# ErickRosete/tacorl

Measured on AMD Instinct MI355X. Metric: offline grad-steps/sec (batch=256, 84x84 RGB), higher is better.
Workload: dtype bf16; 1 GPU; tacorl actor-critic training_step, frozen LMP (BASELINE configs[1]); per_gpu_batch=256, global_batch=256, window=16, image=84x84x3, frames=fp32 CHW (reference batch schema), latent_plan=16, n_action_samples=4, phase=Q (epoch>=bc_epochs), action_decoder_loss=every step (reference behaviour), parallelism=dp1, hip_graph=True, losses_finite=True

## Files before the change

tacorl_amd/csrc/mlp_fused.hip:

```cpp
#include "mlp_fused.h"

#include <stdlib.h>

#include "common.h"

namespace {

constexpr int BMF = 32;
constexpr int MTF = BMF / 16;
constexpr int XP = 272;
constexpr int MAXD = 256;
constexpr int MF_NT = 1024, MF_CW = MAXD / (MF_NT / 64), MF_NTW = MF_CW / 16;

struct MlpXSeg { const float* p; int ld, c0, mod, pad; };
struct MlpFwdArgs {
  MlpXSeg seg[MF_MAXP][MF_MAXSEG];
  int nseg[MF_MAXP];
  float* xw[MF_MAXP];
  const float* x[MF_MAXP];
  const float* params[MF_MAXP];
  const __bf16* pbf[MF_MAXP];
  float* act[MF_MAXP];
  int M[MF_MAXP];
  long zoff[MF_MAXP][MF_MAXL], yoff[MF_MAXP][MF_MAXL];
// ... 375 lines not shown
                if (col + r < KO) o[r] = v[r];
            }
          }
          *reinterpret_cast<bf16x4*>(xout + row * XP + col) = bf16x4{(__bf16)v[0], (__bf16)v[1], (__bf16)v[2], (__bf16)v[3]};
        }
      }
    }
    lds_barrier();
    cur ^= 1;
  }
}
__global__ __launch_bounds__(MF_NT) void mlp_fused_bwd_kernel(MlpBwdArgs a) { mlp_fused_bwd_body<32>(a); }
__global__ __launch_bounds__(MF_NT) void mlp_fused_bwd_big_kernel(MlpBwdArgs a) { mlp_fused_bwd_body<64>(a); }

constexpr int WG_MS = 2048;
constexpr int WG_MT = 32;
constexpr int WG_TP = 40;
constexpr int WG_OPB = 256 * WG_TP * 2;

struct MlpWgArgs {
  const float* x[MF_MAXP];
  const float* act[MF_MAXP];
  const float* dlast[MF_MAXP];
  const float* dz[MF_MAXP];
  float* slab[MF_MAXP];
  int M[MF_MAXP];
  long yoff[MF_MAXP][MF_MAXL], dzoff[MF_MAXP][MF_MAXL];
  int acts[MF_MAXL];
  long sloff[MF_MAXL];
  long rec;
  int dims[MF_MAXL + 1];
  int L, ldx, ldo, ms;
};

__device__ __forceinline__ float wg_dpp1(float x) {
  return __builtin_bit_cast(float, __builtin_amdgcn_mov_dpp(__builtin_bit_cast(int, x), 0xB1, 0xF, 0xF, true));
}
__device__ __forceinline__ float wg_dpp2(float x) {
  return __builtin_bit_cast(float, __builtin_amdgcn_mov_dpp(__builtin_bit_cast(int, x), 0x4E, 0xF, 0xF, true));
}
__device__ __forceinline__ void wg_quad_transpose(f32x4& v, int q) {
  const bool o1 = q & 1, o2 = q & 2;
  const float x0 = wg_dpp1(o1 ? v[0] : v[1]), x1 = wg_dpp1(o1 ? v[2] : v[3]);
  if (o1) { v[0] = x0; v[2] = x1; } else { v[1] = x0; v[3] = x1; }
  const float y0 = wg_dpp2(o2 ? v[0] : v[2]), y1 = wg_dpp2(o2 ? v[1] : v[3]);
  if (o2) { v[0] = y0; v[1] = y1; } else { v[2] = y0; v[3] = y1; }
}

__global__ __launch_bounds__(512) void mlp_wgrad_fused_kernel(MlpWgArgs a) {
  extern __shared__ __attribute__((aligned(16))) unsigned char smem[];
  const int p = blockIdx.z, l = blockIdx.y, m0 = blockIdx.x * a.ms, M = a.M[p];
  if (m0 >= M) return;
  const int tid = threadIdx.x, lane = tid & 63, w = tid >> 6, i = lane & 15, g = lane >> 4, q = tid & 3;
  const int qd = (tid >> 2) & 63, jh = tid >> 8;
  const int K = a.dims[l], N = a.dims[l + 1];
  const long yo = l == 0 ? 0 : a.yoff[p][l - 1];
  const float* X = l == 0 ? a.x[p] : a.act[p] + (yo < 0 ? -(yo + 1) : yo);
  const int actX = l > 0 && yo < 0 ? a.acts[l - 1] : ACT_NONE;
  const int ldX = l == 0 ? a.ldx : K;
  const float* Z = l == a.L - 1 ? a.dlast[p] : a.dz[p] + a.dzoff[p][l];
  const int ldZ = l == a.L - 1 ? a.ldo : N;
  const bool vecX = (ldX & 3) == 0 && (K & 3) == 0 && ((uintptr_t)X & 15) == 0;
  const bool vecZ = (ldZ & 3) == 0 && (N & 3) == 0 && ((uintptr_t)Z & 15) == 0;
  const int KT = (K + 15) >> 4, NT = (N + 15) >> 4;
  const int mend = min(M, m0 + a.ms), nsteps = (mend - m0 + WG_MT - 1) / WG_MT;

  f32x4 rx[4], rz[4];
  auto fetch = [&](const float* S, int ld, int C, bool vec, int mt, f32x4 (&r)[4]) {
    const int c = 4 * qd;
#pragma unroll
    for (int j = 0; j < 4; j++) {
      const int m = m0 + mt * WG_MT + 4 * (2 * j + jh) + q;
      const bool rok = m < mend;
      const float* src = S + (long)(rok ? m : m0) * ld;
      if (vec) {
        const f32x4 v = *reinterpret_cast<const f32x4*>(src + (c < C ? c : 0));
        const bool ok = rok && c < C;
        r[j] = f32x4{ok ? v[0] : 0.f, ok ? v[1] : 0.f, ok ? v[2] : 0.f, ok ? v[3] : 0.f};
      } else {
#pragma unroll
        for (int e = 0; e < 4; e++) {
          const float v = src[c + e < C ? c + e : 0];
          r[j][e] = rok && c + e < C ? v : 0.f;
        }
      }
    }
  };
  auto stash = [&](f32x4 (&r)[4], unsigned char* T, int act) {
#pragma unroll
    for (int j = 0; j < 4; j++) {
      f32x4 v = r[j];
      if (act != ACT_NONE) v = f32x4{act_fast(act, v[0]), act_fast(act, v[1]), act_fast(act, v[2]), act_fast(act, v[3])};
      wg_quad_transpose(v, q);
      *reinterpret_cast<bf16x4*>(T + ((4 * qd + q) * WG_TP + 4 * (2 * j + jh)) * 2) = bf16x4{(__bf16)v[0], (__bf16)v[1], (__bf16)v[2], (__bf16)v[3]};
    }
  };
  f32x4 acc[2][17];
#pragma unroll
  for (int nt = 0; nt < 2; nt++)
#pragma unroll
    for (int kt = 0; kt < 17; kt++) acc[nt][kt] = f32x4{0.f, 0.f, 0.f, 0.f};
  const __bf16 one = (__bf16)1.0f;
  const bf16x8 ones = {one, one, one, one, one, one, one, one};

  fetch(X, ldX, K, vecX, 0, rx);
  fetch(Z, ldZ, N, vecZ, 0, rz);
  for (int s = 0; s < nsteps; s++) {
    unsigned char* TX = smem + (s & 1) * 2 * WG_OPB;
    unsigned char* TZ = TX + WG_OPB;
    stash(rx, TX, actX);
    stash(rz, TZ, ACT_NONE);
    __syncthreads();
    if (s + 1 < nsteps) { fetch(X, ldX, K, vecX, s + 1, rx); fetch(Z, ldZ, N, vecZ, s + 1, rz); }
    bf16x8 zf[2];
#pragma unroll
    for (int nt = 0; nt < 2; nt++)
      zf[nt] = *reinterpret_cast<const bf16x8*>(TZ + ((16 * (w + 8 * nt) + i) * WG_TP + 8 * g) * 2);
#pragma unroll
    for (int kt = 0; kt < 16; kt++) {
      if (kt < KT) {
        const bf16x8 xf = *reinterpret_cast<const bf16x8*>(TX + ((16 * kt + i) * WG_TP + 8 * g) * 2);
#pragma unroll
        for (int nt = 0; nt < 2; nt++)
          if (w + 8 * nt < NT) acc[nt][kt] = __builtin_amdgcn_mfma_f32_16x16x32_bf16(xf, zf[nt], acc[nt][kt], 0, 0, 0);
      }
    }
#pragma unroll
    for (int nt = 0; nt < 2; nt++)
      if (w + 8 * nt < NT) acc[nt][16] = __builtin_amdgcn_mfma_f32_16x16x32_bf16(ones, zf[nt], acc[nt][16], 0, 0, 0);
  }
  float* rec = a.slab[p] + (long)blockIdx.x * a.rec + a.sloff[l];
  const bool vecK = (K & 3) == 0;
#pragma unroll
  for (int nt = 0; nt < 2; nt++) {
    const int n = 16 * (w + 8 * nt) + i;
    if (w + 8 * nt >= NT || n >= N) continue;
#pragma unroll
    for (int kt = 0; kt < 16; kt++) {
      const int k = 16 * kt + 4 * g;
      if (kt < KT) {
        if (vecK) {
          if (k < K) *reinterpret_cast<f32x4*>(rec + (long)n * K + k) = acc[nt][kt];
        } else {
#pragma unroll
          for (int r = 0; r < 4; r++)
            if (k + r < K) rec[(long)n * K + k + r] = acc[nt][kt][r];
        }
      }
    }
    if (g == 0) rec[(long)N * K + n] = acc[nt][16][0];
  }
}

struct MlpWgReduceArgs {
  const float* slab[MF_MAXP];
  float* grad[MF_MAXP];
  int nslice[MF_MAXP];
  long sloff[MF_MAXL], woff[MF_MAXL], boff[MF_MAXL];
  long rec;
  int dims[MF_MAXL + 1];
  int accumulate;
};
__global__ __launch_bounds__(256) void mlp_wgrad_reduce_kernel(MlpWgReduceArgs a) {
  const int l = blockIdx.y, p = blockIdx.z, K = a.dims[l], N = a.dims[l + 1], ns = a.nslice[p];
  const long nw = (long)N * K, tot = nw + N;
  const float* __restrict__ s0 = a.slab[p] + a.sloff[l];
  float* __restrict__ gr = a.grad[p];
  for (long e = (long)blockIdx.x * 256 + threadIdx.x; e < tot; e += (long)gridDim.x * 256) {
    float t = 0.f;
#pragma unroll 8
    for (int s = 0; s < ns; s++) t += s0[(long)s * a.rec + e];
    float* d = gr + (e < nw ? a.woff[l] + e : a.boff[l] + (e - nw));
    *d = a.accumulate ? *d + t : t;
  }
}

#define RED_MAXJ 8
struct MlpWgReduceMulti {
  MlpWgReduceArgs job[RED_MAXJ];
  int gx[RED_MAXJ], L[RED_MAXJ], first[RED_MAXJ + 1];
  int njob;
};
__global__ __launch_bounds__(256) void mlp_wgrad_reduce_multi_kernel(MlpWgReduceMulti m) {
  int j = 0;
#pragma unroll
  for (int t = 1; t < RED_MAXJ; t++) j = (t < m.njob && (int)blockIdx.z >= m.first[t]) ? t : j;
  const int gx = m.gx[j];
  if ((int)blockIdx.y >= m.L[j] || (int)blockIdx.x >= gx) return;
  const MlpWgReduceArgs& a = m.job[j];
  const int l = blockIdx.y, p = blockIdx.z - m.first[j], K = a.dims[l], N = a.dims[l + 1], ns = a.nslice[p];
  const long nw = (long)N * K, tot = nw + N;
  const float* __restrict__ s0 = a.slab[p] + a.sloff[l];
  float* __restrict__ gr = a.grad[p];
  for (long e = (long)blockIdx.x * 256 + threadIdx.x; e < tot; e += (long)gx * 256) {
    float t = 0.f;
#pragma unroll 8
    for (int s = 0; s < ns; s++) t += s0[(long)s * a.rec + e];
    float* d = gr + (e < nw ? a.woff[l] + e : a.boff[l] + (e - nw));
    *d = a.accumulate ? *d + t : t;
  }
}
struct RedState { bool on = false; MlpWgReduceMulti m{}; };
thread_local RedState g_red;
int red_flush(hipStream_t st) {
  MlpWgReduceMulti& m = g_red.m;
  if (m.njob == 0) return 0;
  int gx = 1, Ly = 1;
  for (int j = 0; j < m.njob; j++) { gx = m.gx[j] > gx ? m.gx[j] : gx; Ly = m.L[j] > Ly ? m.L[j] : Ly; }
  hipLaunchKernelGGL(mlp_wgrad_reduce_multi_kernel, dim3(gx, Ly, m.first[m.njob]), dim3(256), 0, st, m);
  m.njob = 0; m.first[0] = 0;
  return hipGetLastError() == hipSuccess ? 0 : -1;
}
int launch_reduce(const MlpWgReduceArgs& r, int gx, int Ly, int nprob, hipStream_t st) {
  if (!g_red.on) {
    hipLaunchKernelGGL(mlp_wgrad_reduce_kernel, dim3(gx, Ly, nprob), dim3(256), 0, st, r);
    return hipGetLastError() == hipSuccess ? 0 : -1;
  }
  MlpWgReduceMulti& m = g_red.m;
  if (m.njob == RED_MAXJ) {
    hipLaunchKernelGGL(mlp_wgrad_reduce_kernel, dim3(gx, Ly, nprob), dim3(256), 0, st, r);
    return hipGetLastError() == hipSuccess ? 0 : -1;
  }
  m.job[m.njob] = r; m.gx[m.njob] = gx; m.L[m.njob] = Ly; m.first[m.njob + 1] = m.first[m.njob] + nprob;
  m.njob++;
  return 0;
}

typedef _Float16 f16x4 __attribute__((ext_vector_type(4)));
#ifdef MLP_STAMPS
__device__ unsigned long long g_mlp_stamps[2][64];
#define MLP_STAMP(k, j) do { if (stamp_on) g_mlp_stamps[k][j] = clock64(); } while (0)
#else
#define MLP_STAMP(k, j) do { } while (0)
#endif

struct MlpBigFwdArgs {
  MlpXSeg seg[MF_MAXP][MF_MAXSEG];
  int nseg[MF_MAXP];
  float* xw[MF_MAXP];
  const float* x[MF_MAXP];
  const float* params[MF_MAXP];
  const __bf16* pbf[MF_MAXP];
  float* act[MF_MAXP];
  int M[MF_MAXP];
  long ybf[MF_MAXP][MF_MAXL], sbf[MF_MAXP][MF_MAXL];
  long yout[MF_MAXP];
  long woff[MF_MAXL], boff[MF_MAXL];
  int dims[MF_MAXL + 1], acts[MF_MAXL];
  int L, ldx;
  int dbg;
};

template <int BMF_>
__device__ __forceinline__ void mlp_big_fwd_body(const MlpBigFwdArgs& a) {
  constexpr int BMF = BMF_, MTF = BMF / 16;
  extern __shared__ __attribute__((aligned(16))) unsigned char smem[];
  __bf16* X = reinterpret_cast<__bf16*>(smem);
  const int p = blockIdx.y, m0 = blockIdx.x * BMF, M = a.M[p];
  const int Mp = (M + 63) & ~63;
  if (m0 >= Mp) return;
  const int tid = threadIdx.x, lane = tid & 63, w = tid >> 6, i = lane & 15, g = lane >> 4;
  const int n0 = MF_CW * w;
#ifdef MLP_STAMPS
  const bool stamp_on = blockIdx.x == 300 && p == 0 && tid == 0;
#endif
  MLP_STAMP(0, 0);
  const int K0 = a.dims[0], c8 = (K0 + 7) / 8;
  f32x4 xr[2][2];
  const float* x = a.x[p];
  const int ns = a.nseg[p];
#pragma unroll
  for (int u = 0; u < 2; u++) {
    const int c = tid + u * MF_NT, row = c / c8, k = (c - row * c8) * 8;
    const bool ok = c < BMF * c8 && m0 + row < M;
    if (ns > 0) {
      int sg = 0;
#pragma unroll
      for (int t = 1; t < MF_MAXSEG; t++) sg = (t < ns && k >= a.seg[p][t].c0) ? t : sg;
      const MlpXSeg s = a.seg[p][sg];
      const int cend = sg + 1 < ns ? a.seg[p][sg + 1].c0 : K0;
      const int r = s.mod ? (m0 + row) % s.mod : m0 + row;
      const float* q = s.p + (ok ? (long)r * s.ld + (k - s.c0) : 0);
      if (ok && k + 8 <= cend) { xr[u][0] = *reinterpret_cast<const f32x4*>(q); xr[u][1] = *reinterpret_cast<const f32x4*>(q + 4); }
      else {
#pragma unroll
        for (int j = 0; j < 4; j++) { xr[u][0][j] = ok && k + j < cend ? q[j] : 0.f; xr[u][1][j] = ok && k + 4 + j < cend ? q[4 + j] : 0.f; }
      }
      continue;
    }
    const float* q = x + (ok ? (long)(m0 + row) * a.ldx + k : 0);
    if (ok && k + 8 <= a.ldx) { xr[u][0] = *reinterpret_cast<const f32x4*>(q); xr[u][1] = *reinterpret_cast<const f32x4*>(q + 4); }
    else {
#pragma unroll
      for (int j = 0; j < 4; j++) { xr[u][0][j] = ok && k + j < K0 ? q[j] : 0.f; xr[u][1][j] = ok && k + 4 + j < K0 ? q[4 + j] : 0.f; }
    }
  }
  bf16x8 B[8][MF_NTW];
  auto load_layer = [&](int l) {
    const int K = a.dims[l], N = a.dims[l + 1];
    const __bf16* Wb = a.pbf[p] + a.woff[l];
#pragma unroll
    for (int ks = 0; ks < 8; ks++)
#pragma unroll
      for (int nt = 0; nt < MF_NTW; nt++) B[ks][nt] = load_w(Wb, K, N, n0 + 16 * nt + i, 32 * ks + 8 * g);
  };
  if (n0 < a.dims[1]) load_layer(0);
// ... 857 lines not shown
      if (k + 8 <= a.ldx && (a.ldx & 3) == 0) {
        const f32x4 lo = *reinterpret_cast<const f32x4*>(q), hi = *reinterpret_cast<const f32x4*>(q + 4);
#pragma unroll
        for (int j = 0; j < 4; j++) { v[j] = (__bf16)(k + j < K0 ? lo[j] : 0.f); v[4 + j] = (__bf16)(k + 4 + j < K0 ? hi[j] : 0.f); }
      } else {
#pragma unroll
        for (int j = 0; j < 8; j++)
          if (k + j < K0) v[j] = (__bf16)q[j];
      }
    }
    *reinterpret_cast<bf16x8*>(o + (long)row * 128 + k) = v;
  }
}

constexpr int OUT_RPW = 512;
struct MlpWgOutArgs {
  const __bf16* y[MF_MAXP]; const float* dlast[MF_MAXP]; float* slab[MF_MAXP];
  int M[MF_MAXP];
  long rec;
  int NL, ldo, rpw;
};
__global__ __launch_bounds__(256) void mlp_wgrad_out_kernel(MlpWgOutArgs a) {
  __shared__ float red[8][4][256 + 1];
  const int p = blockIdx.y, M = a.M[p], r0 = blockIdx.x * a.rpw;
  if (r0 >= M) return;
  const int r1 = min(M, r0 + a.rpw), tid = threadIdx.x, cg = tid & 31, rg = tid >> 5, NL = a.NL;
  float acc[4][8], bsum[4];
#pragma unroll
  for (int n = 0; n < 4; n++) {
    bsum[n] = 0.f;
#pragma unroll
    for (int j = 0; j < 8; j++) acc[n][j] = 0.f;
  }
  const __bf16* __restrict__ y = a.y[p];
  const float* __restrict__ d = a.dlast[p];
  for (int rb = r0 + rg; rb < r1; rb += 32) {
    bf16x8 v[4];
    float dv[4][4];
#pragma unroll
    for (int u = 0; u < 4; u++) {
      const int r = rb + 8 * u, rc = r < r1 ? r : r0;
      v[u] = *reinterpret_cast<const bf16x8*>(y + (long)rc * 256 + 8 * cg);
#pragma unroll
      for (int n = 0; n < 4; n++) dv[u][n] = (n < NL && r < r1) ? (float)(__bf16)d[(long)rc * a.ldo + n] : 0.f;
    }
#pragma unroll
    for (int u = 0; u < 4; u++)
#pragma unroll
      for (int n = 0; n < 4; n++)
        if (n < NL) {
          bsum[n] += dv[u][n];
#pragma unroll
          for (int j = 0; j < 8; j++) acc[n][j] += dv[u][n] * (float)v[u][j];
        }
  }
#pragma unroll
  for (int n = 0; n < 4; n++) {
#pragma unroll
    for (int j = 0; j < 8; j++) red[rg][n][8 * cg + j] = acc[n][j];
    if (cg == 0) red[rg][n][256] = bsum[n];
  }
  __syncthreads();
  float* rec = a.slab[p] + (long)blockIdx.x * a.rec;
  for (int e = tid; e < NL * 257; e += 256) {
    const int n = e / 257, k = e - n * 257;
    float t = 0.f;
#pragma unroll
    for (int g8 = 0; g8 < 8; g8++) t += red[g8][n][k];
    if (k < 256) rec[(long)n * 256 + k] = t; else rec[(long)NL * 256 + n] = t;
  }
}

}

namespace {
struct PrepState {
  bool on = false;
  PrepMultiArgs a{};
  int nprob[PREP_MAXS] = {};
};
thread_local PrepState g_prep;
int prep_flush(hipStream_t st) {
  PrepMultiArgs& a = g_prep.a;
  if (a.nsite == 0 && a.ncv == 0) return TACORL_OK;
  int maxL = 1;
  for (int s = 0; s < a.nsite; s++) maxL = a.site[s].L > maxL ? a.site[s].L : maxL;
  hipLaunchKernelGGL(prep_multi_kernel, dim3(64, maxL, a.first[a.nsite] + a.ncv), dim3(256), 0, st, a);
  a.nsite = 0; a.ncv = 0; a.first[0] = 0;
  return hipGetLastError() == hipSuccess ? TACORL_OK : TACORL_ELAUNCH;
}
}
bool prep_deferring() { return g_prep.on; }
int prep_defer_wtpack(const WtPackArgs& k, int nprob, hipStream_t st) {
  PrepMultiArgs& a = g_prep.a;
  if (a.nsite == PREP_MAXS) { const int rc = prep_flush(st); if (rc != TACORL_OK) return rc; }
  a.site[a.nsite] = k;
  a.first[a.nsite + 1] = a.first[a.nsite] + nprob;
  a.nsite++;
  return TACORL_OK;
}
int prep_defer_bf16(const float* src, void* dst, long count, hipStream_t st) {
  PrepMultiArgs& a = g_prep.a;
  if (a.ncv == PREP_MAXB) { const int rc = prep_flush(st); if (rc != TACORL_OK) return rc; }
  a.csrc[a.ncv] = src; a.cdst[a.ncv] = (__bf16*)dst; a.cn4[a.ncv] = count / 4;
  a.ncv++;
  return TACORL_OK;
}
extern "C" int tacorl_reduce_batch_begin(void) {
  if (g_red.on) return TACORL_EINVAL;
  g_red.on = true;
  g_red.m.njob = 0; g_red.m.first[0] = 0;
  return TACORL_OK;
}
extern "C" int tacorl_reduce_batch_end(void* stream) {
  if (!g_red.on) return TACORL_EINVAL;
  g_red.on = false;
  return red_flush((hipStream_t)stream) ? TACORL_ELAUNCH : TACORL_OK;
}
extern "C" int tacorl_prep_batch_begin(void) {
  if (g_prep.on) return TACORL_EINVAL;
  g_prep.on = true;
  g_prep.a.nsite = 0; g_prep.a.ncv = 0; g_prep.a.first[0] = 0;
  return TACORL_OK;
}
extern "C" int tacorl_prep_batch_end(void* stream) {
  if (!g_prep.on) return TACORL_EINVAL;
  g_prep.on = false;
  return prep_flush((hipStream_t)stream);
}


bool mlp_fused_wgrad_ok(int nprob, int L, const int* dims) {
  if (nprob < 1 || nprob > MF_MAXP || L < 1 || L > MF_MAXL) return false;
  for (int l = 0; l <= L; l++)
    if (dims[l] < 1 || dims[l] > MAXD) return false;
  return true;
}
static long mlp_wgrad_record(int L, const int* dims, long* sloff) {
  long off = 0;
  for (int l = 0; l < L; l++) {
    if (sloff) sloff[l] = off;
    off += (long)dims[l + 1] * dims[l] + dims[l + 1];
    off = (off + 3) & ~3L;
  }
  return off;
}
static int mlp_wgrad_rows(int nprob, const int* M, int L) {
  long rows = 0;
  for (int p = 0; p < nprob; p++) rows += M[p] > 0 ? M[p] : 0;
  long ms = rows * L / 128;
  ms = (ms + WG_MT - 1) / WG_MT * WG_MT;
  return (int)(ms < WG_MT ? WG_MT : ms > WG_MS ? WG_MS : ms);
}
size_t mlp_fused_wgrad_slab_floats(int nprob, const int* M, int L, const int* dims) {
  const long rec = mlp_wgrad_record(L, dims, nullptr);
  const int ms = mlp_wgrad_rows(nprob, M, L);
  size_t tot = 0;
  for (int p = 0; p < nprob; p++) tot += (size_t)((M[p] + ms - 1) / ms) * rec;
  return tot;
}
int mlp_fused_wgrad(int nprob, const float* const* x, int ldx, const float* const* act, const float* const* d_out, int ldo,
                    const float* const* dz, float* const* grads, float* slab, const int* M, int L, const int* dims,
                    const long* yoff, const long* dzoff, const long* woff, const long* boff, int accumulate, hipStream_t st,
                    const int* acts) {
  MlpWgArgs a{};
  MlpWgReduceArgs r{};
  a.rec = r.rec = mlp_wgrad_record(L, dims, a.sloff);
  a.L = L; a.ldx = ldx; a.ldo = ldo; r.accumulate = accumulate;
  {
    int Mg[MF_MAXP], n = 0;
    for (int p = 0; p < nprob; p++) Mg[n++] = M[p];
    a.ms = mlp_wgrad_rows(n, Mg, L);
  }
  for (int l = 0; l <= L; l++) a.dims[l] = r.dims[l] = dims[l];
  for (int l = 0; l < L; l++) { r.sloff[l] = a.sloff[l]; r.woff[l] = woff[l]; r.boff[l] = boff[l]; a.acts[l] = acts ? acts[l] : ACT_NONE; }
  int n2 = 0, maxs = 0;
  float* sp = slab;
  for (int p = 0; p < nprob; p++) {
    if (!grads[p] || M[p] <= 0) continue;
    const int ns = (M[p] + a.ms - 1) / a.ms;
    a.x[n2] = x[p]; a.act[n2] = act[p]; a.dlast[n2] = d_out[p]; a.dz[n2] = dz[p]; a.M[n2] = M[p]; a.slab[n2] = sp;
    r.slab[n2] = sp; r.grad[n2] = grads[p]; r.nslice[n2] = ns;
    for (int l = 0; l < L; l++) { a.yoff[n2][l] = yoff[p * MF_MAXL + l]; a.dzoff[n2][l] = dzoff[p * MF_MAXL + l]; }
    sp += (size_t)ns * a.rec;
    maxs = ns > maxs ? ns : maxs;
    n2++;
  }
  if (!n2) return 0;
  static int once = hipFuncSetAttribute(reinterpret_cast<const void*>(mlp_wgrad_fused_kernel),
                                        hipFuncAttributeMaxDynamicSharedMemorySize, 4 * WG_OPB) == hipSuccess ? 0 : -1;
  if (once) return -1;
  hipLaunchKernelGGL(mlp_wgrad_fused_kernel, dim3(maxs, L, n2), dim3(512), 4 * WG_OPB, st, a);
  if (launch_reduce(r, 256, L, n2, st)) return -1;
  return hipGetLastError() == hipSuccess ? 0 : -1;
}

static int mlp_big_rows() {
  static const int v = [] { const char* e = getenv("TACORL_MLP_BIG_ROWS"); return e ? atoi(e) : 2048; }();
  return v;
}
bool mlp_big_prob_ok(int M, int L, const int* dims, const int* acts) {
  static const int on = [] { const char* e = getenv("TACORL_MLP_BIG"); return e ? atoi(e) : 1; }();
  if (!on || L < 2 || L > MF_MAXL || M < mlp_big_rows()) return false;
  if (dims[0] < 8 || dims[0] > 128 || dims[L] < 1 || dims[L] > 4) return false;
  for (int l = 1; l < L; l++)
    if (dims[l] != 256) return false;
  if (acts) {
    for (int l = 0; l + 1 < L; l++)
      if (acts[l] != ACT_SILU) return false;
    if (acts[L - 1] != ACT_NONE) return false;
  }
  return true;
}
#ifdef MLP_STAMPS
extern "C" int tacorl_dbg_mlp_stamps(unsigned long long* dst) {
  return hipMemcpyFromSymbol(dst, HIP_SYMBOL(g_mlp_stamps), sizeof(g_mlp_stamps)) == hipSuccess ? 0 : -1;
}
#endif
static bool mlp_rows_huge(int maxM) { return maxM >= 16384; }
static int mlp_env_int(const char* name, int dflt) { const char* e = getenv(name); return e ? atoi(e) : dflt; }
static int mlp_huge_fwd_rows() { static const int v = mlp_env_int("TACORL_MLP_HUGE_FWD_ROWS", 128); return v; }
static int mlp_huge_bwd_rows() { static const int v = mlp_env_int("TACORL_MLP_HUGE_BWD_ROWS", 64); return v; }
template <class Args>
static int mlp_set_gather(Args& a, int p, int q, const MlpXGather* gather, int K0) {
  const int ns = gather ? gather->nseg[q] : 0;
  if (ns < 0 || ns > MF_MAXSEG) return TACORL_EINVAL;
  a.nseg[p] = ns;
  a.xw[p] = ns ? gather->xw[q] : nullptr;
  if ((uintptr_t)a.xw[p] & 15) return TACORL_EINVAL;
  for (int t = 0; t < ns; t++) {
    const int c0 = gather->c0[q][t], ld = gather->ld[q][t];
    if (((uintptr_t)gather->ptr[q][t] & 15) || !gather->ptr[q][t] || ld % 4 || c0 % 8 || (t == 0 ? c0 != 0 : c0 <= gather->c0[q][t - 1]) ||
        c0 >= K0 || gather->mod[q][t] < 0)
      return TACORL_EINVAL;
    a.seg[p][t] = MlpXSeg{gather->ptr[q][t], ld, c0, gather->mod[q][t], 0};
  }
  return TACORL_OK;
}
int mlp_big_fwd(int nprob, const float* const* x, int ldx, const float* const* params, const void* const* params_bf16,
                float* const* act, const int* M, int L, const int* dims, const int* acts, const long* ybf, const long* sbf,
                const long* yout, const long* woff, const long* boff, hipStream_t st, const MlpXGather* gather, const int* gmap) {
  MlpBigFwdArgs a{};
  int maxM = 0;
  for (int p = 0; p < nprob; p++) {
    if (mlp_set_gather(a, p, gmap ? gmap[p] : p, gather, dims[0]) != TACORL_OK) return TACORL_EINVAL;
    if ((!a.nseg[p] && ((uintptr_t)x[p] & 15)) || ((uintptr_t)params[p] & 15) || ((uintptr_t)params_bf16[p] & 7) || ((uintptr_t)act[p] & 15)) return TACORL_EINVAL;
    a.x[p] = x[p]; a.params[p] = params[p]; a.pbf[p] = (const __bf16*)params_bf16[p]; a.act[p] = act[p]; a.M[p] = M[p];
    for (int l = 0; l < L; l++) { a.ybf[p][l] = ybf[p * MF_MAXL + l]; a.sbf[p][l] = sbf[p * MF_MAXL + l]; }
    a.yout[p] = yout[p];
    maxM = M[p] > maxM ? M[p] : maxM;
  }
  for (int l = 0; l < L; l++) {
    if (woff[l] % 4) return TACORL_EINVAL;
    a.woff[l] = woff[l]; a.boff[l] = boff[l]; a.dims[l] = dims[l]; a.acts[l] = acts[l];
  }
  a.dims[L] = dims[L]; a.L = L; a.ldx = ldx;
  if (maxM == 0) return TACORL_OK;
  constexpr size_t lds = (size_t)2 * 128 * XP * 2, lds_mid = (size_t)2 * 32 * XP * 2, lds_64 = (size_t)2 * 64 * XP * 2;
  static int once = (hipFuncSetAttribute(reinterpret_cast<const void*>(mlp_big_fwd_kernel),
                                         hipFuncAttributeMaxDynamicSharedMemorySize, (int)lds) == hipSuccess &&
                     hipFuncSetAttribute(reinterpret_cast<const void*>(mlp_m64_fwd_kernel),
                                         hipFuncAttributeMaxDynamicSharedMemorySize, (int)lds_64) == hipSuccess &&
                     hipFuncSetAttribute(reinterpret_cast<const void*>(mlp_mid_fwd_kernel),
                                         hipFuncAttributeMaxDynamicSharedMemorySize, (int)lds_mid) == hipSuccess) ? 0 : -1;
  if (once) return TACORL_ELAUNCH;
  const int maxMp = (maxM + 63) & ~63;
  {
    const char* pe = getenv("TACORL_MLP_PERS");
    bool pers = mlp_rows_huge(maxM) && (pe ? atoi(pe) : 1) && (L == 3 || L == 4) && dims[0] <= 32 * PF_K0S && dims[L] <= 4;
    for (int l = 0; l + 1 < L && pers; l++) pers = acts[l] == ACT_SILU && dims[l + 1] == 256;
    if (pers) {
      { const char* de = getenv("TACORL_MLP_PERS_DBG"); a.dbg = de ? atoi(de) : 0; }
      static int once_p = (hipFuncSetAttribute(reinterpret_cast<const void*>(mlp_pers_fwd_kernel<1>),
                                               hipFuncAttributeMaxDynamicSharedMemorySize, PF_LDS) == hipSuccess &&
                           hipFuncSetAttribute(reinterpret_cast<const void*>(mlp_pers_fwd_kernel<2>),
                                               hipFuncAttributeMaxDynamicSharedMemorySize, PF_LDS) == hipSuccess) ? 0 : -1;
      if (once_p) return TACORL_ELAUNCH;
      static const int ncu = [] { int d = 0, n = 0; if (hipGetDevice(&d) != hipSuccess || hipDeviceGetAttribute(&n, hipDeviceAttributeMultiprocessorCount, d) != hipSuccess || n < 1) n = 256; return n; }();
      const char* ce = getenv("TACORL_MLP_PERS_CUS");
      int gx = (ce && atoi(ce) > 0 && atoi(ce) < ncu ? atoi(ce) : ncu) / nprob;
      gx = gx < 1 ? 1 : gx;
      gx = gx > maxMp / PF_BM ? maxMp / PF_BM : gx;
      if (L == 3) hipLaunchKernelGGL(mlp_pers_fwd_kernel<1>, dim3(gx, nprob), dim3(PF_NT), PF_LDS, st, a);
      else hipLaunchKernelGGL(mlp_pers_fwd_kernel<2>, dim3(gx, nprob), dim3(PF_NT), PF_LDS, st, a);
      return hipGetLastError() == hipSuccess ? TACORL_OK : TACORL_ELAUNCH;
    }
  }
  const int rows = mlp_rows_huge(maxM) ? mlp_huge_fwd_rows() : 32;
  if (rows == 128) hipLaunchKernelGGL(mlp_big_fwd_kernel, dim3((maxMp + 127) / 128, nprob), dim3(MF_NT), lds, st, a);
  else if (rows == 64) hipLaunchKernelGGL(mlp_m64_fwd_kernel, dim3(maxMp / 64, nprob), dim3(MF_NT), lds_64, st, a);
  else hipLaunchKernelGGL(mlp_mid_fwd_kernel, dim3(maxMp / 32, nprob), dim3(MF_NT), lds_mid, st, a);
  return hipGetLastError() == hipSuccess ? TACORL_OK : TACORL_ELAUNCH;
}
int mlp_big_bwd(int nprob, const float* const* act, const float* const* d_out, int ldo, float* const* dz, float* const* d_x,
                int ldd, void* const* wt, const int* M, int L, const int* dims, const long* sbf, const long* dzoff,
                hipStream_t st) {
  MlpBigBwdArgs a{};
  long wtoff[MF_MAXL];
  mlp_fused_wt_elems(L, dims, wtoff);
  int maxM = 0;
  for (int p = 0; p < nprob; p++) {
    if (((uintptr_t)wt[p] | (uintptr_t)dz[p] | (uintptr_t)act[p]) & 15) return TACORL_EINVAL;
    a.d_out[p] = d_out[p]; a.act[p] = act[p]; a.wt[p] = (const __bf16*)wt[p]; a.dz[p] = dz[p];
    a.d_x[p] = d_x ? d_x[p] : nullptr; a.M[p] = M[p];
    for (int l = 0; l < L; l++) { a.sbf[p][l] = sbf[p * MF_MAXL + l]; a.dzoff[p][l] = dzoff[p * MF_MAXL + l]; }
    maxM = M[p] > maxM ? M[p] : maxM;
  }
  for (int l = 0; l < L; l++) a.wtoff[l] = wtoff[l];
  for (int l = 0; l <= L; l++) a.dims[l] = dims[l];
  a.L = L; a.ldo = ldo; a.ldd = ldd;
  if (maxM == 0) return TACORL_OK;
  constexpr size_t lds = (size_t)3 * 64 * XP * 2, lds_mid = (size_t)3 * 32 * XP * 2;
  static int once = (hipFuncSetAttribute(reinterpret_cast<const void*>(mlp_big_bwd_kernel),
                                         hipFuncAttributeMaxDynamicSharedMemorySize, (int)lds) == hipSuccess &&
                     hipFuncSetAttribute(reinterpret_cast<const void*>(mlp_mid_bwd_kernel),
                                         hipFuncAttributeMaxDynamicSharedMemorySize, (int)lds_mid) == hipSuccess) ? 0 : -1;
  if (once) return TACORL_ELAUNCH;
// ... 206 lines not shown
```

Before: 1233 grad-steps/s.

## Add single-pass banded MLP weight-gradient kernel for small row counts

Adds a weight-gradient kernel in which each block owns a 64-wide output band of one layer and loops over all rows itself. It double-buffers swizzled bf16 tiles in LDS and accumulates dW and the bias gradient with MFMA, writing the result directly. This replaces the split-M slab write plus separate reduce kernel when every problem has at most 512 rows. The cost is less parallelism, since only one block per band runs through all of M, plus a large dynamic shared-memory footprint. The new path is on by default and can be disabled with an environment variable or when g_red is on.

```diff
diff --git a/tacorl_amd/csrc/mlp_fused.hip b/tacorl_amd/csrc/mlp_fused.hip
--- a/tacorl_amd/csrc/mlp_fused.hip
+++ b/tacorl_amd/csrc/mlp_fused.hip
@@ -551,6 +551,147 @@
   }
 }
 
+constexpr int WB_NB = 64;
+constexpr int WB_TS = 2;
+constexpr int WB_XB = 256 * 64;
+constexpr int WB_ZB = WB_NB * 64;
+constexpr int WB_BUF = WB_TS * (WB_XB + WB_ZB);
+__device__ __forceinline__ int wb_sw(int col) { return ((col >> 2) & 1) | ((((col >> 2) ^ (col >> 3)) & 1) << 1); }
+constexpr int WB_MAXM = 512;
+
+struct MlpWgBandArgs {
+  const float* x[MF_MAXP];
+  const float* act[MF_MAXP];
+  const float* dlast[MF_MAXP];
+  const float* dz[MF_MAXP];
+  float* grad[MF_MAXP];
+  int M[MF_MAXP];
+  long yoff[MF_MAXP][MF_MAXL], dzoff[MF_MAXP][MF_MAXL];
+  int acts[MF_MAXL];
+  long woff[MF_MAXL], boff[MF_MAXL];
+  int dims[MF_MAXL + 1];
+  int L, ldx, ldo, accumulate;
+};
+
+__global__ __launch_bounds__(512) void mlp_wgrad_band_kernel(MlpWgBandArgs a) {
+  extern __shared__ __attribute__((aligned(16))) unsigned char smem[];
+  const int p = blockIdx.z, l = blockIdx.y, n0 = blockIdx.x * WB_NB, M = a.M[p];
+  const int K = a.dims[l], N = a.dims[l + 1];
+  if (n0 >= N || M <= 0) return;
+  const int tid = threadIdx.x, lane = tid & 63, w = tid >> 6, i = lane & 15, g = lane >> 4, q = lane & 3;
+  const int cq = (lane >> 2) & 3, jh = (lane >> 4) & 1, hi = lane >> 5;
+  const int qd = 8 * w + 4 * hi + cq;
+  const int zq = 4 * (w & 3) + cq, zj = 2 * (w >> 2) + hi;
+  const int nt = w & 3, kh = w >> 2;
+  const long yo = l == 0 ? 0 : a.yoff[p][l - 1];
+  const float* X = l == 0 ? a.x[p] : a.act[p] + (yo < 0 ? -(yo + 1) : yo);
+  const int actX = l > 0 && yo < 0 ? a.acts[l - 1] : ACT_NONE;
+  const int ldX = l == 0 ? a.ldx : K;
+  const float* Z = l == a.L - 1 ? a.dlast[p] : a.dz[p] + a.dzoff[p][l];
+  const int ldZ = l == a.L - 1 ? a.ldo : N;
+  const bool vecX = (ldX & 3) == 0 && (K & 3) == 0 && ((uintptr_t)X & 15) == 0;
+  const bool vecZ = (ldZ & 3) == 0 && (N & 3) == 0 && ((uintptr_t)Z & 15) == 0;
+  const int KT = (K + 15) >> 4, NTb = (min(N - n0, WB_NB) + 15) >> 4;
+  const int nsteps = (M + WB_TS * WG_MT - 1) / (WB_TS * WG_MT);
+
+  auto load4 = [&](const float* S, int ld, int C, bool vec, int m, int c) {
+    const bool rok = m < M;
+    const float* src = S + (long)(rok ? m : 0) * ld;
+    f32x4 r;
+    if (vec) {
+      const f32x4 v = *reinterpret_cast<const f32x4*>(src + (c < C ? c : 0));
+      const bool ok = rok && c < C;
+      r = f32x4{ok ? v[0] : 0.f, ok ? v[1] : 0.f, ok ? v[2] : 0.f, ok ? v[3] : 0.f};
+    } else {
+#pragma unroll
+      for (int e = 0; e < 4; e++) {
+        const float v = src[c + e < C ? c + e : 0];
+        r[e] = rok && c + e < C ? v : 0.f;
+      }
+    }
+    return r;
+  };
+  f32x4 rx[WB_TS][4], rz[WB_TS];
+  auto fetch = [&](int s) {
+#pragma unroll
+    for (int t = 0; t < WB_TS; t++) {
+      const int mb = (s * WB_TS + t) * WG_MT;
+#pragma unroll
+      for (int j = 0; j < 4; j++) rx[t][j] = load4(X, ldX, K, vecX, mb + 4 * (2 * j + jh) + q, 4 * qd);
+      rz[t] = load4(Z, ldZ, N, vecZ, mb + 4 * (2 * zj + jh) + q, n0 + 4 * zq);
+    }
+  };
+  auto put = [&](f32x4 v, unsigned char* T, int col, int row) {
+    wg_quad_transpose(v, q);
+    *reinterpret_cast<bf16x4*>(T + col * 64 + 16 * ((row >> 3) ^ wb_sw(col)) + 2 * (row & 7)) = bf16x4{(__bf16)v[0], (__bf16)v[1], (__bf16)v[2], (__bf16)v[3]};
+  };
+  f32x4 acc[9];
+#pragma unroll
+  for (int u = 0; u < 9; u++) acc[u] = f32x4{0.f, 0.f, 0.f, 0.f};
+  const __bf16 one = (__bf16)1.0f;
+  const bf16x8 ones = {one, one, one, one, one, one, one, one};
+
+  fetch(0);
+  for (int s = 0; s < nsteps; s++) {
+    unsigned char* buf = smem + (s & 1) * WB_BUF;
+#pragma unroll
+    for (int t = 0; t < WB_TS; t++) {
+      unsigned char* TX = buf + t * (WB_XB + WB_ZB);
+#pragma unroll
+      for (int j = 0; j < 4; j++) {
+        f32x4 v = rx[t][j];
+        if (actX != ACT_NONE) v = f32x4{act_fast(actX, v[0]), act_fast(actX, v[1]), act_fast(actX, v[2]), act_fast(actX, v[3])};
+        put(v, TX, 4 * qd + q, 4 * (2 * j + jh));
+      }
+      put(rz[t], TX + WB_XB, 4 * zq + q, 4 * (2 * zj + jh));
+    }
+    __syncthreads();
+    if (s + 1 < nsteps) fetch(s + 1);
+#pragma unroll
+    for (int t = 0; t < WB_TS; t++) {
+      const unsigned char* TX = buf + t * (WB_XB + WB_ZB);
+      const int fo = i * 64 + 16 * (g ^ wb_sw(i));
+      const bf16x8 zf = *reinterpret_cast<const bf16x8*>(TX + WB_XB + nt * 1024 + fo);
+#pragma unroll
+      for (int u = 0; u < 8; u++) {
+        const int kt = 2 * u + kh;
+        if (kt < KT && nt < NTb) {
+          const bf16x8 xf = *reinterpret_cast<const bf16x8*>(TX + kt * 1024 + fo);
+          acc[u] = __builtin_amdgcn_mfma_f32_16x16x32_bf16(xf, zf, acc[u], 0, 0, 0);
+        }
+      }
+      if (kh == 0 && nt < NTb) acc[8] = __builtin_amdgcn_mfma_f32_16x16x32_bf16(ones, zf, acc[8], 0, 0, 0);
+    }
+  }
+  const int n = n0 + 16 * nt + i;
+  if (nt >= NTb || n >= N) return;
+  float* dW = a.grad[p] + a.woff[l];
+  const bool vecK = (K & 3) == 0 && ((uintptr_t)dW & 15) == 0;
+  const bool accu = a.accumulate != 0;
+#pragma unroll
+  for (int u = 0; u < 8; u++) {
+    const int kt = 2 * u + kh, k = 16 * kt + 4 * g;
+    if (kt < KT) {
+      float* d = dW + (long)n * K + k;
+      if (vecK) {
+        if (k < K) {
+          f32x4 v = acc[u];
+          if (accu) { const f32x4 o = *reinterpret_cast<const f32x4*>(d); v = f32x4{o[0] + v[0], o[1] + v[1], o[2] + v[2], o[3] + v[3]}; }
+          *reinterpret_cast<f32x4*>(d) = v;
+        }
+      } else {
+#pragma unroll
+        for (int r = 0; r < 4; r++)
+          if (k + r < K) d[r] = accu ? d[r] + acc[u][r] : acc[u][r];
+      }
+    }
+  }
+  if (kh == 0 && g == 0) {
+    float* d = a.grad[p] + a.boff[l] + n;
+    *d = accu ? *d + acc[8][0] : acc[8][0];
+  }
+}
+
 struct MlpWgReduceArgs {
   const float* slab[MF_MAXP];
   float* grad[MF_MAXP];
@@ -1714,6 +1855,14 @@
   ms = (ms + WG_MT - 1) / WG_MT * WG_MT;
   return (int)(ms < WG_MT ? WG_MT : ms > WG_MS ? WG_MS : ms);
 }
+static bool mlp_wgrad_band_rows(int nprob, const int* M) {
+  if (g_red.on) return false;
+  const char* e = getenv("TACORL_MLP_WGRAD_BAND");
+  if (e && atoi(e) == 0) return false;
+  for (int p = 0; p < nprob; p++)
+    if (M[p] > WB_MAXM) return false;
+  return true;
+}
 size_t mlp_fused_wgrad_slab_floats(int nprob, const int* M, int L, const int* dims) {
   const long rec = mlp_wgrad_record(L, dims, nullptr);
   const int ms = mlp_wgrad_rows(nprob, M, L);
@@ -1725,6 +1874,25 @@
                     const float* const* dz, float* const* grads, float* slab, const int* M, int L, const int* dims,
                     const long* yoff, const long* dzoff, const long* woff, const long* boff, int accumulate, hipStream_t st,
                     const int* acts) {
+  if (mlp_wgrad_band_rows(nprob, M)) {
+    MlpWgBandArgs b{};
+    b.L = L; b.ldx = ldx; b.ldo = ldo; b.accumulate = accumulate;
+    for (int l = 0; l <= L; l++) b.dims[l] = dims[l];
+    int n2 = 0, maxN = 0;
+    for (int l = 0; l < L; l++) { b.woff[l] = woff[l]; b.boff[l] = boff[l]; b.acts[l] = acts ? acts[l] : ACT_NONE; maxN = dims[l + 1] > maxN ? dims[l + 1] : maxN; }
+    for (int p = 0; p < nprob; p++) {
+      if (!grads[p] || M[p] <= 0) continue;
+      b.x[n2] = x[p]; b.act[n2] = act[p]; b.dlast[n2] = d_out[p]; b.dz[n2] = dz[p]; b.M[n2] = M[p]; b.grad[n2] = grads[p];
+      for (int l = 0; l < L; l++) { b.yoff[n2][l] = yoff[p * MF_MAXL + l]; b.dzoff[n2][l] = dzoff[p * MF_MAXL + l]; }
+      n2++;
+    }
+    if (!n2) return 0;
+    static int once = hipFuncSetAttribute(reinterpret_cast<const void*>(mlp_wgrad_band_kernel),
+                                          hipFuncAttributeMaxDynamicSharedMemorySize, 2 * WB_BUF) == hipSuccess ? 0 : -1;
+    if (once) return -1;
+    hipLaunchKernelGGL(mlp_wgrad_band_kernel, dim3((maxN + WB_NB - 1) / WB_NB, L, n2), dim3(512), 2 * WB_BUF, st, b);
+    return hipGetLastError() == hipSuccess ? 0 : -1;
+  }
   MlpWgArgs a{};
   MlpWgReduceArgs r{};
   a.rec = r.rec = mlp_wgrad_record(L, dims, a.sloff);
```

After: 1169 grad-steps/s. 0.949x the previous value.
